# google/TensorNetwork

Hardware: NVIDIA H100
Metric: pairwise contractions/s (higher is better)
Workload: dtype bf16

## Files before the change

tensornetwork_b200/csrc/tensordot_thin.cu:

```cuda
#include "common.cuh"
#include <algorithm>
#include <vector>

namespace tnb {

struct ThinParams {
  const void* X; const void* S; void* C;
  int64_t L;
  int K, P;
  int64_t sXl, sXk;
  int64_t sCl;
  int64_t sSk;
  int64_t bX, bS, bC;
  int64_t batch;
  DevModes mP;
};

enum ThinKind { THIN_SIMT = 0, THIN_MMA = 1, THIN_MMA_TF32 = 2 };

template <typename T> struct Vec16 { static constexpr int N = 16 / (int)sizeof(T); };

__device__ __forceinline__ uint4 ldg16(const void* p) { return __ldg(reinterpret_cast<const uint4*>(p)); }

template <typename T> struct alignas(16) Pack16 { T v[Vec16<T>::N]; };

template <typename T, typename Acc, int KK, int PP>
__device__ __forceinline__ void simt_a_unit(const Acc (&w)[KK][PP], const Pack16<T> (&x)[KK], int K, int P, T* cp,
                                            const long long (&co)[PP]) {
  constexpr int VE = Vec16<T>::N;
  Acc acc[PP][VE];
#pragma unroll
  for (int i = 0; i < PP; ++i)
#pragma unroll
    for (int v = 0; v < VE; ++v) acc[i][v] = acc_zero((Acc*)nullptr);
#pragma unroll
  for (int k = 0; k < KK; ++k)
    if (k < K) {
#pragma unroll
      for (int v = 0; v < VE; ++v) {
        const Acc xv = to_acc(x[k].v[v]);
#pragma unroll
        for (int i = 0; i < PP; ++i) fma_acc(acc[i][v], w[k][i], xv);
      }
    }
#pragma unroll
  for (int i = 0; i < PP; ++i)
    if (i < P) {
      Pack16<T> o;
#pragma unroll
      for (int v = 0; v < VE; ++v) o.v[v] = FromAcc<T, Acc>::f(acc[i][v]);
      *reinterpret_cast<uint4*>(cp + co[i]) = *reinterpret_cast<uint4*>(&o);
    }
}

template <typename T, typename Acc, int KK, int PP>
__global__ void __launch_bounds__(256) thin_simt_a_kernel(const __grid_constant__ ThinParams p) {
  constexpr int VE = Vec16<T>::N;
  constexpr int U = (KK * PP <= 16) ? 2 : 1;
  __shared__ __align__(16) Acc sS[KK][PP];
  __shared__ long long cOff[PP];
  const int64_t bb = blockIdx.y;
  const T* Xb = (const T*)p.X + bb * p.bX;
  const T* Sb = (const T*)p.S + bb * p.bS;
  T* Cb = (T*)p.C + bb * p.bC;
  if (threadIdx.x < KK * PP) {
    const int k = threadIdx.x / PP, pp = threadIdx.x % PP;
    Acc v = acc_zero((Acc*)nullptr);
    if (pp < p.P) {
      int64_t os, oc;
      mode_offsets(p.mP, pp, os, oc);
      if (k < p.K) v = to_acc(Sb[os + k * p.sSk]);
      if (k == 0) cOff[pp] = oc;
    }
    sS[k][pp] = v;
  }
  __syncthreads();
  Acc w[KK][PP];
#pragma unroll
  for (int k = 0; k < KK; ++k)
#pragma unroll
    for (int i = 0; i < PP; ++i) w[k][i] = sS[k][i];
  long long co[PP];
#pragma unroll
  for (int i = 0; i < PP; ++i) co[i] = i < p.P ? cOff[i] : 0;
  const int64_t nunits = p.L / VE;
  const int64_t stride = (int64_t)gridDim.x * blockDim.x;
  for (int64_t u0 = blockIdx.x * (int64_t)blockDim.x + threadIdx.x; u0 < nunits; u0 += stride * U) {
    Pack16<T> x[U][KK];
#pragma unroll
    for (int j = 0; j < U; ++j)
      if (u0 + j * stride < nunits) {
        const T* xp = Xb + (u0 + j * stride) * VE;
#pragma unroll
        for (int k = 0; k < KK; ++k)
          if (k < p.K) *reinterpret_cast<uint4*>(&x[j][k]) = ldg16(xp + k * p.sXk);
      }
#pragma unroll
    for (int j = 0; j < U; ++j)
      if (u0 + j * stride < nunits) simt_a_unit<T, Acc, KK, PP>(w, x[j], p.K, p.P, Cb + (u0 + j * stride) * VE, co);
  }
}

template <typename T, int KK, int PP> struct SimtD {
  static constexpr int VE = Vec16<T>::N;
  static constexpr int UE = VE > KK ? VE : KK;
  static constexpr int R = UE / KK;
  static constexpr int NV = UE / VE;
  static constexpr int OE = R * PP;
  static constexpr int OB = OE * (int)sizeof(T);
};

template <typename T, typename Acc, int KK, int PP>
__device__ __forceinline__ void simt_d_unit(const Acc (&w)[KK][PP], const Pack16<T> (&x)[SimtD<T, KK, PP>::NV], T* cp) {
  using G = SimtD<T, KK, PP>;
  constexpr int VE = G::VE, R = G::R, OE = G::OE, OB = G::OB;
  struct alignas(OB >= 16 ? 16 : OB) Out { T v[OE]; };
  Out o;
#pragma unroll
  for (int r = 0; r < R; ++r) {
    Acc acc[PP];
#pragma unroll
    for (int j = 0; j < PP; ++j) acc[j] = acc_zero((Acc*)nullptr);
#pragma unroll
    for (int k = 0; k < KK; ++k) {
      const int e = r * KK + k;
      const Acc xv = to_acc(x[e / VE].v[e % VE]);
#pragma unroll
      for (int j = 0; j < PP; ++j) fma_acc(acc[j], xv, w[k][j]);
    }
#pragma unroll
    for (int j = 0; j < PP; ++j) o.v[r * PP + j] = FromAcc<T, Acc>::f(acc[j]);
  }
  if constexpr (OB >= 16) {
#pragma unroll
    for (int v = 0; v < OB / 16; ++v) reinterpret_cast<uint4*>(cp)[v] = reinterpret_cast<uint4*>(&o)[v];
  } else if constexpr (OB == 8) {
    *reinterpret_cast<uint2*>(cp) = *reinterpret_cast<uint2*>(&o);
  } else if constexpr (OB == 4) {
    *reinterpret_cast<uint32_t*>(cp) = *reinterpret_cast<uint32_t*>(&o);
  } else {
#pragma unroll
    for (int v = 0; v < OE; ++v) cp[v] = o.v[v];
  }
}

template <typename T, typename Acc, int KK, int PP>
__global__ void __launch_bounds__(256) thin_simt_d_kernel(const __grid_constant__ ThinParams p) {
  using G = SimtD<T, KK, PP>;
  constexpr int VE = G::VE, UE = G::UE, NV = G::NV, OE = G::OE;
  __shared__ Acc sS[KK][PP];
  const int64_t bb = blockIdx.y;
  const T* Xb = (const T*)p.X + bb * p.bX;
  const T* Sb = (const T*)p.S + bb * p.bS;
  T* Cb = (T*)p.C + bb * p.bC;
// ... 215 lines not shown
  const T* Sb = (const T*)p.S + bb * p.bS;
  T* Cb = (T*)p.C + bb * p.bC;
  for (int idx = threadIdx.x; idx < PP * KK; idx += blockDim.x) {
    const int pp = idx / KK, k = idx % KK;
    T v = FromAcc<T, float>::f(0.f);
    if (pp < p.P) {
      int64_t os, oc;
      mode_offsets(p.mP, pp, os, oc);
      v = Sb[os + k * p.sSk];
      if (k == 0) cOff[pp] = oc;
    }
    sS[pp * PITCH + k] = v;
  }
  __syncthreads();
  const int lane = threadIdx.x & 31, warp = threadIdx.x >> 5;
  const int g = lane >> 2, q = lane & 3;
  const int64_t nblk = p.L >> 6;
  const int64_t wstride = (int64_t)gridDim.x * (blockDim.x >> 5);

  if constexpr (MODE == 0) {
    uint32_t sa[PT][KT][4];
    mma_a_frags<T, KT, PT>(sS, sa, g, q);
    const int colbase = 32 * (g & 1) + 8 * (g >> 1);
    for (int64_t blk = (int64_t)blockIdx.x * (blockDim.x >> 5) + warp; blk < nblk; blk += wstride) {
      const int64_t l0 = blk << 6;
      mma_a_block<T, KT, PT, true>(sa, Xb + l0 + colbase, p.sXk, Cb + l0 + 8 * q, cOff, p.P, g, q);
    }
  } else {
    uint32_t sb[KT][2 * PT][2];
    mma_d_frags<T, KT, PT>(sS, sb, g, q);
    for (int64_t blk = (int64_t)blockIdx.x * (blockDim.x >> 5) + warp; blk < nblk; blk += wstride) {
      const int64_t l0 = blk << 6;
      mma_d_block<T, KT, PT, true>(sb, Xb + l0 * p.sXl, p.sXl, Cb + l0 * p.sCl, p.sCl, g, q);
    }
  }
}


__device__ __forceinline__ void mma_tf32(float (&d)[4], const uint32_t (&a)[4], uint32_t b0, uint32_t b1) {
  asm volatile("mma.sync.aligned.m16n8k8.row.col.f32.tf32.tf32.f32 {%0,%1,%2,%3}, {%4,%5,%6,%7}, {%8,%9}, {%0,%1,%2,%3};"
               : "+f"(d[0]), "+f"(d[1]), "+f"(d[2]), "+f"(d[3])
               : "r"(a[0]), "r"(a[1]), "r"(a[2]), "r"(a[3]), "r"(b0), "r"(b1));
}

template <int KT8, int PT, int MODE>
__global__ void __launch_bounds__(256) thin_mma32_kernel(const __grid_constant__ ThinParams p) {
  constexpr int KK = 8 * KT8, PP = 16 * PT, PITCH = KK + 4;
  __shared__ __align__(16) float sS[PP * PITCH];
  __shared__ long long cOff[PP];
  const int64_t bb = blockIdx.y;
  const float* Xb = (const float*)p.X + bb * p.bX;
  const float* Sb = (const float*)p.S + bb * p.bS;
  float* Cb = (float*)p.C + bb * p.bC;
  for (int idx = threadIdx.x; idx < PP * KK; idx += blockDim.x) {
    const int pp = idx / KK, k = idx % KK;
    float v = 0.f;
    if (pp < p.P) {
      int64_t os, oc;
      mode_offsets(p.mP, pp, os, oc);
      v = Sb[os + k * p.sSk];
      if (k == 0) cOff[pp] = oc;
    }
    sS[pp * PITCH + k] = v;
  }
  __syncthreads();
  const int lane = threadIdx.x & 31, warp = threadIdx.x >> 5;
  const int g = lane >> 2, q = lane & 3;
  const int64_t wstride = (int64_t)gridDim.x * (blockDim.x >> 5);

  if constexpr (MODE == 0) {
    const int64_t nblk = p.L >> 5;
    const int colbase = 16 * (g & 1) + 4 * (g >> 1);
    for (int64_t blk = (int64_t)blockIdx.x * (blockDim.x >> 5) + warp; blk < nblk; blk += wstride) {
      const int64_t l0 = blk << 5;
      const float* xp = Xb + l0 + colbase;
      uint4 x[KT8][2];
#pragma unroll
      for (int t = 0; t < KT8; ++t)
#pragma unroll
        for (int h = 0; h < 2; ++h) x[t][h] = ldg16(xp + (int64_t)(8 * t + q + 4 * h) * p.sXk);
#pragma unroll
      for (int mt = 0; mt < PT; ++mt) {
        if (16 * mt >= p.P) break;
        float acc[4][4];
#pragma unroll
        for (int j = 0; j < 4; ++j) { acc[j][0] = acc[j][1] = acc[j][2] = acc[j][3] = 0.f; }
#pragma unroll
        for (int t = 0; t < KT8; ++t) {
          const float* r0 = sS + (16 * mt + g) * PITCH + 8 * t + q;
          const uint32_t a[4] = {__float_as_uint(r0[0]), __float_as_uint(r0[8 * PITCH]), __float_as_uint(r0[4]),
                                 __float_as_uint(r0[8 * PITCH + 4])};
          mma_tf32(acc[0], a, x[t][0].x, x[t][1].x);
          mma_tf32(acc[1], a, x[t][0].y, x[t][1].y);
          mma_tf32(acc[2], a, x[t][0].z, x[t][1].z);
          mma_tf32(acc[3], a, x[t][0].w, x[t][1].w);
        }
#pragma unroll
        for (int h = 0; h < 2; ++h) {
          const int row = 16 * mt + g + 8 * h;
          if (row < p.P) {
            float* cp = Cb + cOff[row] + l0 + 4 * q;
            *reinterpret_cast<float4*>(cp) = make_float4(acc[0][2 * h], acc[1][2 * h], acc[2][2 * h], acc[3][2 * h]);
            *reinterpret_cast<float4*>(cp + 16) = make_float4(acc[0][2 * h + 1], acc[1][2 * h + 1], acc[2][2 * h + 1], acc[3][2 * h + 1]);
          }
        }
      }
    }
  } else {
    constexpr int NP8 = 2 * PT;
    constexpr int RG = KT8 == 8 ? 2 : 4;
    const int64_t nblk = p.L / (16 * RG);
    for (int64_t blk = (int64_t)blockIdx.x * (blockDim.x >> 5) + warp; blk < nblk; blk += wstride) {
      const int64_t l0 = blk * (16 * RG);
      uint32_t xa[RG][2][2 * KT8];
#pragma unroll
      for (int rg = 0; rg < RG; ++rg)
#pragma unroll
        for (int h = 0; h < 2; ++h) {
          const float* rp = Xb + (l0 + 16 * rg + 8 * h + g) * p.sXl + 2 * KT8 * q;
#pragma unroll
          for (int v4 = 0; v4 < KT8 / 2; ++v4) {
            const uint4 v = ldg16(rp + 4 * v4);
            xa[rg][h][4 * v4] = v.x; xa[rg][h][4 * v4 + 1] = v.y; xa[rg][h][4 * v4 + 2] = v.z; xa[rg][h][4 * v4 + 3] = v.w;
          }
        }
#pragma unroll
      for (int rg = 0; rg < RG; ++rg) {
        float acc[NP8][4];
#pragma unroll
        for (int pt = 0; pt < NP8; ++pt) { acc[pt][0] = acc[pt][1] = acc[pt][2] = acc[pt][3] = 0.f; }
#pragma unroll
        for (int t = 0; t < KT8; ++t) {
          const uint32_t a[4] = {xa[rg][0][2 * t], xa[rg][1][2 * t], xa[rg][0][2 * t + 1], xa[rg][1][2 * t + 1]};
#pragma unroll
          for (int pt = 0; pt < NP8; ++pt) {
            const int pcol = (pt >> 1) * 16 + 4 * (g >> 1) + 2 * (pt & 1) + (g & 1);
            const float2 b = *reinterpret_cast<const float2*>(sS + pcol * PITCH + 2 * KT8 * q + 2 * t);
            mma_tf32(acc[pt], a, __float_as_uint(b.x), __float_as_uint(b.y));
          }
        }
#pragma unroll
        for (int h = 0; h < 2; ++h) {
          float* cp = Cb + (l0 + 16 * rg + 8 * h + g) * p.sCl + 4 * q;
#pragma unroll
          for (int piece = 0; piece < NP8 / 2; ++piece)
            *reinterpret_cast<float4*>(cp + 16 * piece) =
                make_float4(acc[2 * piece][2 * h], acc[2 * piece][2 * h + 1], acc[2 * piece + 1][2 * h], acc[2 * piece + 1][2 * h + 1]);
        }
      }
    }
  }
}

constexpr int kRunMaxSteps = 8, kRunWarps = 8, kRunSlab = 4096;

struct ThinRunStep {
  const void* S; int64_t bS, sSk;
  int K, P, kind;
  int W;
  int64_t L;
  int soff;
};
struct ThinRunParams {
  const void* X; void* C;
  int64_t sX, bX;
  int64_t sC, bC;
  int64_t batch, nslab;
  int nsteps, smem_s;
  const long long* tab;
  ThinRunStep st[kRunMaxSteps];
};

__device__ __forceinline__ int run_pt(int P) { return (P + 15) / 16 <= 1 ? 1 : ((P + 15) / 16 <= 2 ? 2 : 4); }

__device__ __forceinline__ int64_t run_col(const ThinRunParams& p, int64_t slab, int n) {
  int64_t l = slab * 64;
  for (int j = p.nsteps - 2; j >= 0; --j) { l += (int64_t)(n / p.st[j].W) * p.st[j].L; n %= p.st[j].W; }
  return l + n;
}

template <typename T, int KT, int PT, int MODE>
__device__ __forceinline__ void run_mma(const ThinRunParams& p, int j, const unsigned char* smem, const long long* cOff,
                                        const T* x, int64_t sX, T* c, int64_t sC, bool last, int64_t slab, int g, int q) {
  const ThinRunStep& st = p.st[j];
  const T* sS = reinterpret_cast<const T*>(smem + st.soff);
  if constexpr (MODE == 0) {
    uint32_t sa[PT][KT][4];
    mma_a_frags<T, KT, PT>(sS, sa, g, q);
    const int colbase = 32 * (g & 1) + 8 * (g >> 1);
    for (int n0 = 0; n0 < st.W; n0 += 64)
      mma_a_block<T, KT, PT, false>(sa, x + n0 + colbase, sX, c + (last ? run_col(p, slab, n0) : n0) + 8 * q, cOff,
                                    st.P, g, q);
  } else {
    uint32_t sb[KT][2 * PT][2];
    mma_d_frags<T, KT, PT>(sS, sb, g, q);
    for (int n0 = 0; n0 < st.W; n0 += 64) mma_d_block<T, KT, PT, false>(sb, x + n0 * sX, sX, c + n0 * sC, sC, g, q);
  }
}

template <typename T, int KK, int PP, int MODE>
__device__ __forceinline__ void run_simt(const ThinRunParams& p, int j, const unsigned char* smem, const long long* cOff,
                                         const T* x, int64_t sX, T* c, bool last, int64_t slab, int lane) {
  using Acc = float;
  constexpr int VE = Vec16<T>::N;
  const ThinRunStep& st = p.st[j];
  const Acc* sS = reinterpret_cast<const Acc*>(smem + st.soff);
  Acc w[KK][PP];
#pragma unroll
  for (int k = 0; k < KK; ++k)
#pragma unroll
    for (int i = 0; i < PP; ++i) w[k][i] = sS[k * PP + i];
  if constexpr (MODE == 0) {
    long long co[PP];
#pragma unroll
    for (int i = 0; i < PP; ++i) co[i] = cOff[i];
    for (int u = lane; u < st.W / VE; u += 32) {
      Pack16<T> xv[KK];
#pragma unroll
      for (int k = 0; k < KK; ++k) *reinterpret_cast<uint4*>(&xv[k]) = ld16<false>(x + k * sX + u * VE);
      simt_a_unit<T, Acc, KK, PP>(w, xv, KK, PP, c + (last ? run_col(p, slab, u * VE) : u * VE), co);
    }
  } else {
    using G = SimtD<T, KK, PP>;
    for (int u = lane; u < st.W * KK / G::UE; u += 32) {
      Pack16<T> xv[G::NV];
#pragma unroll
      for (int v = 0; v < G::NV; ++v) *reinterpret_cast<uint4*>(&xv[v]) = ld16<false>(x + u * G::UE + v * VE);
      simt_d_unit<T, Acc, KK, PP>(w, xv, c + u * G::OE);
    }
  }
}

template <typename T, int MODE>
__global__ void __launch_bounds__(256, 1) thin_run_kernel(const __grid_constant__ ThinRunParams p) {
  extern __shared__ __align__(16) unsigned char smem[];
  long long* cOff = reinterpret_cast<long long*>(smem + p.smem_s);
  T* bufs = reinterpret_cast<T*>(cOff + kRunMaxSteps * 64);
  for (int i = threadIdx.x; i < p.nsteps * 64; i += blockDim.x) cOff[i] = p.tab[(i / 64) * 128 + 64 + i % 64];
  const int lane = threadIdx.x & 31, warp = threadIdx.x >> 5;
  const int g = lane >> 2, q = lane & 3;
  T* const wbuf = bufs + warp * 2 * kRunSlab;
  const int64_t total = p.batch * p.nslab;
  const int64_t beg = total * blockIdx.x / gridDim.x, end = total * (blockIdx.x + 1) / gridDim.x;
  for (int64_t s0 = beg; s0 < end;) {
    const int64_t b = s0 / p.nslab;
    const int64_t s1 = (b + 1) * p.nslab < end ? (b + 1) * p.nslab : end;
    __syncthreads();
    for (int j = 0; j < p.nsteps; ++j) {
      const ThinRunStep& st = p.st[j];
      const T* Sb = (const T*)st.S + b * st.bS;
      const long long* sOff = p.tab + j * 128;
      if (st.kind == THIN_MMA) {
        T* sS = reinterpret_cast<T*>(smem + st.soff);
        const int PP = 16 * run_pt(st.P), pitch = st.K + 8;
        for (int idx = threadIdx.x; idx < PP * st.K; idx += blockDim.x) {
          const int pp = idx / st.K, k = idx % st.K;
          sS[pp * pitch + k] = pp < st.P ? Sb[sOff[pp] + k * st.sSk] : FromAcc<T, float>::f(0.f);
        }
      } else {
        float* sS = reinterpret_cast<float*>(smem + st.soff);
        for (int idx = threadIdx.x; idx < st.K * st.P; idx += blockDim.x) {
          const int k = idx / st.P, pp = idx % st.P;
          sS[idx] = to_acc(Sb[sOff[pp] + k * st.sSk]);
        }
      }
    }
    __syncthreads();
    for (int64_t it = s0 + warp; it < s1; it += kRunWarps) {
      const int64_t slab = it - b * p.nslab;
      for (int j = 0; j < p.nsteps; ++j) {
        const ThinRunStep& st = p.st[j];
        const bool first = j == 0, last = j == p.nsteps - 1;
        const T* x = first ? (const T*)p.X + b * p.bX + slab * 64 * (MODE == 0 ? 1 : p.sX) : wbuf + ((j - 1) & 1) * kRunSlab;
        const int64_t sX = first ? p.sX : (MODE == 0 ? st.W : st.K);
        T* c = last ? (T*)p.C + b * p.bC + (MODE == 0 ? 0 : slab * st.W * p.sC) : wbuf + (j & 1) * kRunSlab;
        const int64_t sC = last ? p.sC : st.P;
        const long long* co = cOff + j * 64;
        if (st.kind == THIN_MMA) {
          const int kt = st.K / 16, pt = run_pt(st.P);
#define TNB_RUN_M(KT, PT) \
  if (kt == KT && pt == PT) run_mma<T, KT, PT, MODE>(p, j, smem, co, x, sX, c, sC, last, slab, g, q); else
          TNB_RUN_M(1, 1) TNB_RUN_M(1, 2) TNB_RUN_M(1, 4) TNB_RUN_M(2, 1) TNB_RUN_M(2, 2) TNB_RUN_M(2, 4)
          TNB_RUN_M(4, 1) TNB_RUN_M(4, 2) TNB_RUN_M(4, 4) {}
#undef TNB_RUN_M
        } else {
#define TNB_RUN_S(KK, PP) \
  if (st.K == KK && st.P == PP) run_simt<T, KK, PP, MODE>(p, j, smem, co, x, sX, c, last, slab, lane); else
          TNB_RUN_S(2, 2) TNB_RUN_S(2, 4) TNB_RUN_S(2, 8) TNB_RUN_S(4, 2) TNB_RUN_S(4, 4) TNB_RUN_S(4, 8)
          TNB_RUN_S(8, 2) TNB_RUN_S(8, 4) TNB_RUN_S(8, 8) {}
#undef TNB_RUN_S
        }
        __syncwarp();
      }
    }
    s0 = s1;
  }
}

static inline unsigned thin_grid_x(int64_t work_items, int64_t batch, int ctas_per_sm) {
  int64_t want = ((int64_t)num_sms() * ctas_per_sm + batch - 1) / batch;
  int64_t cap = (work_items + 255) / 256;
  if (want > cap) want = cap;
  if (want < 1) want = 1;
  return (unsigned)want;
}

template <int DT>
static int launch_simt(int mode, const ThinParams& p, cudaStream_t st) {
  using T = typename DType<DT>::T;
  using Acc = typename DType<DT>::Acc;
  constexpr int VE = 16 / (int)sizeof(T);
  if (mode == 0) {
    const int kk = p.K <= 2 ? 2 : (p.K <= 4 ? 4 : 8), pp = p.P <= 2 ? 2 : (p.P <= 4 ? 4 : 8);
    dim3 grid(thin_grid_x(p.L / VE, p.batch, 8), (unsigned)p.batch);
#define TNB_THIN_A(KK, PP) if (kk == KK && pp == PP) thin_simt_a_kernel<T, Acc, KK, PP><<<grid, 256, 0, st>>>(p);
    TNB_THIN_A(2, 2) TNB_THIN_A(2, 4) TNB_THIN_A(2, 8)
    TNB_THIN_A(4, 2) TNB_THIN_A(4, 4) TNB_THIN_A(4, 8)
    TNB_THIN_A(8, 2) TNB_THIN_A(8, 4) TNB_THIN_A(8, 8)
#undef TNB_THIN_A
    TNB_LAUNCH_CHECK();
    count_launch();
    set_kernel_name("thin_simt_a");
    return 0;
  }
#define TNB_THIN_D(KK, PP)                                                                         \
  if (p.K == KK && p.P == PP) {                                                                    \
    constexpr int UE = VE > KK ? VE : KK;                                                          \
    dim3 grid(thin_grid_x(p.L * KK / UE / 4, p.batch, 8), (unsigned)p.batch);                      \
    thin_simt_d_kernel<T, Acc, KK, PP><<<grid, 256, 0, st>>>(p);                                   \
    TNB_LAUNCH_CHECK();                                                                            \
    count_launch();                                                                                \
    set_kernel_name("thin_simt_d");                                                                \
    return 0;                                                                                      \
  }
  TNB_THIN_D(2, 2) TNB_THIN_D(2, 4) TNB_THIN_D(2, 8)
  TNB_THIN_D(4, 2) TNB_THIN_D(4, 4) TNB_THIN_D(4, 8)
  TNB_THIN_D(8, 2) TNB_THIN_D(8, 4) TNB_THIN_D(8, 8)
#undef TNB_THIN_D
  return TNB200_ERR_UNSUPPORTED;
}

template <int DT, int KT, int PT>
static int launch_mma_kp(int mode, const ThinParams& p, cudaStream_t st) {
  using T = typename DType<DT>::T;
  const int ctas = (KT * PT >= 8) ? 1 : (KT * PT >= 4 ? 2 : 4);
  int64_t want = ((int64_t)num_sms() * ctas + p.batch - 1) / p.batch;
  const int64_t cap = ((p.L >> 6) + 7) / 8;
  if (want > cap) want = cap;
  if (want < 1) want = 1;
  dim3 grid((unsigned)want, (unsigned)p.batch);
  if (mode == 0) thin_mma_kernel<T, KT, PT, 0><<<grid, 256, 0, st>>>(p);
  else thin_mma_kernel<T, KT, PT, 1><<<grid, 256, 0, st>>>(p);
  TNB_LAUNCH_CHECK();
  count_launch();
  set_kernel_name(mode == 0 ? "thin_mma_a" : "thin_mma_d");
  return 0;
}
template <int DT>
static int launch_mma(int mode, const ThinParams& p, cudaStream_t st) {
  const int kt = p.K / 16, pt = (p.P + 15) / 16 <= 1 ? 1 : ((p.P + 15) / 16 <= 2 ? 2 : 4);
#define TNB_THIN_M(KT, PT) if (kt == KT && pt == PT) return launch_mma_kp<DT, KT, PT>(mode, p, st);
  TNB_THIN_M(1, 1) TNB_THIN_M(1, 2) TNB_THIN_M(1, 4)
  TNB_THIN_M(2, 1) TNB_THIN_M(2, 2) TNB_THIN_M(2, 4)
  TNB_THIN_M(4, 1) TNB_THIN_M(4, 2) TNB_THIN_M(4, 4)
#undef TNB_THIN_M
  return TNB200_ERR_UNSUPPORTED;
}

template <int KT8, int PT>
static int launch_mma32_kp(int mode, const ThinParams& p, cudaStream_t st) {
  const int ctas = (KT8 * PT >= 16) ? 2 : 4;
  const int64_t nblk = mode == 0 ? (p.L >> 5) : p.L / (16 * (KT8 == 8 ? 2 : 4));
  int64_t want = ((int64_t)num_sms() * ctas + p.batch - 1) / p.batch;
  const int64_t cap = (nblk + 7) / 8;
  if (want > cap) want = cap;
  if (want < 1) want = 1;
  dim3 grid((unsigned)want, (unsigned)p.batch);
  if (mode == 0) thin_mma32_kernel<KT8, PT, 0><<<grid, 256, 0, st>>>(p);
  else thin_mma32_kernel<KT8, PT, 1><<<grid, 256, 0, st>>>(p);
  TNB_LAUNCH_CHECK();
  count_launch();
  set_kernel_name(mode == 0 ? "thin_mma_tf32_a" : "thin_mma_tf32_d");
  return 0;
}
static int launch_mma32(int mode, const ThinParams& p, cudaStream_t st) {
  const int kt = p.K / 8, pt = (p.P + 15) / 16 <= 1 ? 1 : ((p.P + 15) / 16 <= 2 ? 2 : 4);
#define TNB_THIN_M32(KT8, PT) if (kt == KT8 && pt == PT) return launch_mma32_kp<KT8, PT>(mode, p, st);
  TNB_THIN_M32(2, 1) TNB_THIN_M32(2, 2) TNB_THIN_M32(2, 4)
  TNB_THIN_M32(4, 1) TNB_THIN_M32(4, 2) TNB_THIN_M32(4, 4)
  TNB_THIN_M32(8, 1) TNB_THIN_M32(8, 2) TNB_THIN_M32(8, 4)
#undef TNB_THIN_M32
  return TNB200_ERR_UNSUPPORTED;
}

static inline bool al16(const void* p) { return ((uintptr_t)p & 15) == 0; }

static int plan_thin(int dt, const void* A, const void* B, void* C, const ModeList& mB, const ModeList& mM,
                     const ModeList& mN, const ModeList& mK, bool allow_tf32, ThinParams& p, int& mode, int& kind) {
  if (dt != TNB200_F64 && dt != TNB200_F32 && dt != TNB200_F16 && dt != TNB200_BF16) return TNB200_ERR_UNSUPPORTED;
  if (mB.n > 1 || mK.n != 1) return TNB200_ERR_UNSUPPORTED;
  const int64_t M = mM.total(), N = mN.total(), K = mK.total(), batch = mB.total();
  if (K > 64 || batch > 65535) return TNB200_ERR_UNSUPPORTED;
  const int64_t ve = 16 / dtype_size(dt);
  const bool half_t = dt == TNB200_F16 || dt == TNB200_BF16;
  memset(&p, 0, sizeof(p));
  p.K = (int)K; p.batch = batch;
  mode = -1;
  if (M <= 64 && mN.n == 1 && mN.s0[0] == 1 && mN.s1[0] == 1 && N >= 2048) {
    mode = 0;
    p.X = B; p.S = A; p.C = C; p.L = N; p.P = (int)M;
    p.sXl = 1; p.sXk = mK.s1[0]; p.sSk = mK.s0[0]; p.sCl = 1;
    p.bX = mB.n ? mB.s1[0] : 0; p.bS = mB.n ? mB.s0[0] : 0; p.bC = mB.n ? mB.s2[0] : 0;
    ModeList sp;
    for (int i = 0; i < mM.n; ++i) sp.push(mM.ext[i], mM.s0[i], mM.s1[i]);
    if (!to_dev(sp, p.mP)) return TNB200_ERR_UNSUPPORTED;
    bool ok = al16(B) && al16(C) && p.sXk % ve == 0 && p.bX % ve == 0 && p.bC % ve == 0;
    for (int i = 0; i < mM.n && ok; ++i) ok = mM.s1[i] % ve == 0;
    if (!ok) return TNB200_ERR_UNSUPPORTED;
  } else if (N <= 64 && mM.n == 1 && mK.s0[0] == 1 && M >= 2048) {
    int64_t run = 1;
    for (int i = mN.n - 1; i >= 0; --i) { if (mN.s1[i] != run) return TNB200_ERR_UNSUPPORTED; run *= mN.ext[i]; }
    mode = 1;
    p.X = A; p.S = B; p.C = C; p.L = M; p.P = (int)N;
    p.sXl = mM.s0[0]; p.sXk = 1; p.sSk = mK.s1[0]; p.sCl = mM.s1[0];
    p.bX = mB.n ? mB.s0[0] : 0; p.bS = mB.n ? mB.s1[0] : 0; p.bC = mB.n ? mB.s2[0] : 0;
    ModeList sp;
    for (int i = 0; i < mN.n; ++i) sp.push(mN.ext[i], mN.s0[i], mN.s1[i]);
    if (!to_dev(sp, p.mP)) return TNB200_ERR_UNSUPPORTED;
    if (!(al16(A) && al16(C) && p.bX % ve == 0 && p.bC % ve == 0)) return TNB200_ERR_UNSUPPORTED;
  } else {
    return TNB200_ERR_UNSUPPORTED;
  }
  if (p.L * batch < 65536) return TNB200_ERR_UNSUPPORTED;
  if (K <= 8 && p.P <= 8) {
    if (mode == 0) {
      if (p.L % ve) return TNB200_ERR_UNSUPPORTED;
    } else {
      const int64_t ue = ve > K ? ve : K;
      if (p.sXl != K || p.sCl != p.P || (p.L * K) % ue) return TNB200_ERR_UNSUPPORTED;
      if (!((K == 2 || K == 4 || K == 8) && (p.P == 2 || p.P == 4 || p.P == 8))) return TNB200_ERR_UNSUPPORTED;
    }
    kind = THIN_SIMT;
    return 0;
  }
  if (half_t && (K == 16 || K == 32 || K == 64) && p.P > 8 && p.L % 64 == 0) {
    if (mode == 1) {
      if (!(p.P == 16 || p.P == 32 || p.P == 64)) return TNB200_ERR_UNSUPPORTED;
      if (p.sXl % 8 || p.sCl % 8) return TNB200_ERR_UNSUPPORTED;
    }
    kind = THIN_MMA;
    return 0;
  }
  if (dt == TNB200_F32 && allow_tf32 && (K == 16 || K == 32 || K == 64) && p.P > 8) {
    if (mode == 0) {
      if (p.L % 32) return TNB200_ERR_UNSUPPORTED;
    } else {
      if (!(p.P == 16 || p.P == 32 || p.P == 64)) return TNB200_ERR_UNSUPPORTED;
      if (p.sXl % 4 || p.sCl % 4 || p.L % 64) return TNB200_ERR_UNSUPPORTED;
    }
    kind = THIN_MMA_TF32;
    return 0;
  }
  return TNB200_ERR_UNSUPPORTED;
}

int tensordot_thin(int dt, const void* A, const void* B, void* C, const ModeList& mB, const ModeList& mM,
                   const ModeList& mN, const ModeList& mK, bool allow_tf32, cudaStream_t st) {
  ThinParams p;
  int mode, kind;
  const int rc = plan_thin(dt, A, B, C, mB, mM, mN, mK, allow_tf32, p, mode, kind);
  if (rc) return rc;
  if (kind == THIN_MMA_TF32) return launch_mma32(mode, p, st);
  if (kind == THIN_MMA) return dt == TNB200_F16 ? launch_mma<TNB200_F16>(mode, p, st) : launch_mma<TNB200_BF16>(mode, p, st);
  switch (dt) {
    case TNB200_F64: return launch_simt<TNB200_F64>(mode, p, st);
    case TNB200_F32: return launch_simt<TNB200_F32>(mode, p, st);
    case TNB200_F16: return launch_simt<TNB200_F16>(mode, p, st);
    default: return launch_simt<TNB200_BF16>(mode, p, st);
  }
}

struct ThinRun {
  int dt, mode;
  ThinParams first, last;
  ThinRunParams rp;
  size_t smem;
  int grid;
};

static void host_mode_offsets(const DevModes& m, int64_t lin, int64_t& o0, int64_t& o1) {
  o0 = 0; o1 = 0;
  for (int i = m.n - 1; i > 0; --i) {
    const int64_t q = lin / m.ext[i], r = lin - q * m.ext[i];
    o0 += r * m.s0[i]; o1 += r * m.s1[i];
    lin = q;
  }
  if (m.n > 0) { o0 += lin * m.s0[0]; o1 += lin * m.s1[0]; }
}

template <typename T, int MODE> static void* thin_run_fn() { return (void*)thin_run_kernel<T, MODE>; }
static void* thin_run_kernel_ptr(int dt, int mode) {
  if (dt == TNB200_F16) return mode == 0 ? thin_run_fn<__half, 0>() : thin_run_fn<__half, 1>();
  return mode == 0 ? thin_run_fn<__nv_bfloat16, 0>() : thin_run_fn<__nv_bfloat16, 1>();
}

int thin_run_create(int dt, int nsteps, const ModeList* mB, const ModeList* mM, const ModeList* mN, const ModeList* mK,
                    const void* const* A, const void* const* B, void* const* C, const int* dep_a, const int* dep_b,
                    int* bad, void** handle) {
  *bad = -1;
  if (nsteps < 2 || nsteps > kRunMaxSteps) return TNB200_ERR_UNSUPPORTED;
  if (dt != TNB200_F16 && dt != TNB200_BF16) { *bad = 0; return TNB200_ERR_UNSUPPORTED; }
  std::vector<ThinParams> ps((size_t)nsteps);
  std::vector<long long> tab((size_t)nsteps * 128, 0);
  ThinRun* r = new ThinRun();
  memset(&r->rp, 0, sizeof(r->rp));
  r->dt = dt;
  int W = 64, soff = 0;
  auto fail = [&](int j) { *bad = j; delete r; return TNB200_ERR_UNSUPPORTED; };
  for (int j = 0; j < nsteps; ++j) {
    ThinParams& p = ps[j];
    int mode, kind;
    if (plan_thin(dt, A[j], B[j], C[j], mB[j], mM[j], mN[j], mK[j], false, p, mode, kind)) return fail(j);
    if (j == 0) r->mode = mode;
    if (mode != r->mode || (kind != THIN_SIMT && kind != THIN_MMA)) return fail(j);
    const int dep_x = mode == 0 ? dep_b[j] : dep_a[j], dep_s = mode == 0 ? dep_a[j] : dep_b[j];
    if (dep_s >= 0 || dep_x != j - 1) return fail(j);
    if (kind == THIN_SIMT && !((p.K == 2 || p.K == 4 || p.K == 8) && (p.P == 2 || p.P == 4 || p.P == 8))) return fail(j);
    if (j == 0 && p.L % 64) return fail(0);
    if (j > 0) {
      const ThinParams& pv = ps[j - 1];
      if (p.batch != pv.batch || p.L % pv.L) return fail(j);
      const int64_t R = p.L / pv.L;
      if ((int64_t)pv.P != p.K * R) return fail(j);
      if (r->mode == 0) {
        if (p.sXk < p.L) return fail(j);
        std::vector<char> seen((size_t)pv.P, 0);
        for (int pp = 0; pp < pv.P; ++pp) {
          int64_t os, oc;
          host_mode_offsets(pv.mP, pp, os, oc);
          const int64_t k = oc / p.sXk, rem = oc % p.sXk;
          if (rem % pv.L || rem / pv.L >= R || seen[k * R + rem / pv.L]) return fail(j);
          seen[k * R + rem / pv.L] = 1;
          tab[(size_t)(j - 1) * 128 + 64 + pp] = k * (W * R) + (rem / pv.L) * W;
        }
      } else if (p.sXl != p.K || pv.sCl != pv.P) {
        return fail(j);
      }
      W *= (int)R;
    }
    if ((int64_t)p.K * W > kRunSlab || (int64_t)p.P * W > kRunSlab) return fail(j);
    for (int pp = 0; pp < p.P; ++pp) {
      int64_t os, oc;
      host_mode_offsets(p.mP, pp, os, oc);
      tab[(size_t)j * 128 + pp] = os;
      if (j == nsteps - 1) tab[(size_t)j * 128 + 64 + pp] = oc;
    }
    ThinRunStep& st = r->rp.st[j];
    st.S = p.S; st.bS = p.bS; st.sSk = p.sSk; st.K = p.K; st.P = p.P; st.kind = kind; st.W = W; st.L = p.L;
    st.soff = soff;
    const int pt = (p.P + 15) / 16 <= 1 ? 1 : ((p.P + 15) / 16 <= 2 ? 2 : 4);
    soff += kind == THIN_MMA ? 16 * pt * (p.K + 8) * 2 : p.K * p.P * 4;
    soff = (soff + 15) / 16 * 16;
  }
  const ThinParams &p0 = ps[0], &pl = ps[nsteps - 1];
  ThinRunParams& rp = r->rp;
  rp.X = p0.X; rp.C = pl.C;
  rp.sX = r->mode == 0 ? p0.sXk : p0.sXl; rp.bX = p0.bX;
  rp.sC = pl.sCl; rp.bC = pl.bC;
  rp.batch = p0.batch; rp.nslab = p0.L / 64;
  rp.nsteps = nsteps; rp.smem_s = soff;
  r->smem = (size_t)soff + kRunMaxSteps * 64 * sizeof(long long) + (size_t)kRunWarps * 2 * kRunSlab * 2;
  void* fn = thin_run_kernel_ptr(dt, r->mode);
  int blocks = 0;
  constexpr int kRunSmemMax = kRunMaxSteps * 64 * (64 + 8) * 2 + kRunMaxSteps * 64 * (int)sizeof(long long) +
                              kRunWarps * 2 * kRunSlab * 2;
  if (cudaFuncSetAttribute(fn, cudaFuncAttributeMaxDynamicSharedMemorySize, kRunSmemMax) != cudaSuccess ||
      cudaOccupancyMaxActiveBlocksPerMultiprocessor(&blocks, fn, 256, r->smem) != cudaSuccess || blocks < 1) {
    cudaGetLastError();
    delete r;
    return TNB200_ERR_UNSUPPORTED;
  }
  const int64_t items = (rp.batch * rp.nslab + kRunWarps - 1) / kRunWarps;
  r->grid = (int)std::min<int64_t>((int64_t)blocks * num_sms(), items);
  long long* dtab = nullptr;
  if (cudaMalloc(&dtab, tab.size() * sizeof(long long)) != cudaSuccess ||
      cudaMemcpy(dtab, tab.data(), tab.size() * sizeof(long long), cudaMemcpyHostToDevice) != cudaSuccess) {
    cudaGetLastError();
    if (dtab) cudaFree(dtab);
    delete r;
    return TNB200_ERR_CUDA;
  }
  rp.tab = dtab;
  *handle = r;
  return 0;
}

int thin_run_launch(void* handle, cudaStream_t st) {
  const ThinRun* r = (const ThinRun*)handle;
  if (r->dt == TNB200_F16) {
    if (r->mode == 0) thin_run_kernel<__half, 0><<<r->grid, 256, r->smem, st>>>(r->rp);
    else thin_run_kernel<__half, 1><<<r->grid, 256, r->smem, st>>>(r->rp);
  } else {
    if (r->mode == 0) thin_run_kernel<__nv_bfloat16, 0><<<r->grid, 256, r->smem, st>>>(r->rp);
    else thin_run_kernel<__nv_bfloat16, 1><<<r->grid, 256, r->smem, st>>>(r->rp);
  }
  TNB_LAUNCH_CHECK();
  count_launch();
  set_kernel_name("thin_run");
  return 0;
}

int thin_run_destroy(void* handle) {
  ThinRun* r = (ThinRun*)handle;
  if (!r) return 0;
  cudaFree((void*)r->rp.tab);
  delete r;
  return 0;
}

}
```

Before: 1.158 million.

## Pipeline thin-run chain with cp.async prefetch, double-buffered S staging, and ramp specialization

Restructures the fused multi-step thin contraction kernel. Each warp's first-step input slab is now prefetched into shared memory with cp.async while the remaining chain steps of the previous slab run. The small S operands are staged for two batches at once when shared memory allows, which cuts block-wide barriers. A compile-time specialized 'ramp' variant is added for a K=64,32,16,8,4 halving chain, so dispatch and column-index math are resolved at compile time. This costs an extra warp buffer and more shared memory per block and more template instantiations, and it adds optional timing instrumentation behind a macro.

After: 1.173 million, median of 6. 1.01x the previous value.

```diff
diff --git a/tensornetwork_b200/csrc/tensordot_thin.cu b/tensornetwork_b200/csrc/tensordot_thin.cu
--- a/tensornetwork_b200/csrc/tensordot_thin.cu
+++ b/tensornetwork_b200/csrc/tensordot_thin.cu
@@ -1,5 +1,6 @@
 #include "common.cuh"
 #include <algorithm>
+#include <utility>
 #include <vector>
 
 namespace tnb {
@@ -521,7 +522,7 @@
   }
 }
 
-constexpr int kRunMaxSteps = 8, kRunWarps = 8, kRunSlab = 4096;
+constexpr int kRunMaxSteps = 8, kRunWarps = 8, kRunSlab = 4096, kRunBufs = 3;
 
 struct ThinRunStep {
   const void* S; int64_t bS, sSk;
@@ -536,19 +537,29 @@
   int64_t sC, bC;
   int64_t batch, nslab;
   int nsteps, smem_s;
+  int nsb;
   const long long* tab;
   ThinRunStep st[kRunMaxSteps];
 };
 
 __device__ __forceinline__ int run_pt(int P) { return (P + 15) / 16 <= 1 ? 1 : ((P + 15) / 16 <= 2 ? 2 : 4); }
 
+template <int RAMP>
 __device__ __forceinline__ int64_t run_col(const ThinRunParams& p, int64_t slab, int n) {
   int64_t l = slab * 64;
-  for (int j = p.nsteps - 2; j >= 0; --j) { l += (int64_t)(n / p.st[j].W) * p.st[j].L; n %= p.st[j].W; }
-  return l + n;
-}
-
-template <typename T, int KT, int PT, int MODE>
+  if constexpr (RAMP) {
+    constexpr int NS = __builtin_ctz(RAMP / 4) + 1;
+    for (int j = p.nsteps - 2; j >= NS - 1; --j) { l += (int64_t)(n / p.st[j].W) * p.st[j].L; n %= p.st[j].W; }
+#pragma unroll
+    for (int j = 0; j < NS - 1; ++j) l += (int64_t)((n >> (6 + j)) & 1) * p.st[j].L;
+    return l + (n & 63);
+  } else {
+    for (int j = p.nsteps - 2; j >= 0; --j) { l += (int64_t)(n / p.st[j].W) * p.st[j].L; n %= p.st[j].W; }
+    return l + n;
+  }
+}
+
+template <typename T, int KT, int PT, int MODE, int RAMP>
 __device__ __forceinline__ void run_mma(const ThinRunParams& p, int j, const unsigned char* smem, const long long* cOff,
                                         const T* x, int64_t sX, T* c, int64_t sC, bool last, int64_t slab, int g, int q) {
   const ThinRunStep& st = p.st[j];
@@ -558,7 +569,7 @@
     mma_a_frags<T, KT, PT>(sS, sa, g, q);
     const int colbase = 32 * (g & 1) + 8 * (g >> 1);
     for (int n0 = 0; n0 < st.W; n0 += 64)
-      mma_a_block<T, KT, PT, false>(sa, x + n0 + colbase, sX, c + (last ? run_col(p, slab, n0) : n0) + 8 * q, cOff,
+      mma_a_block<T, KT, PT, false>(sa, x + n0 + colbase, sX, c + (last ? run_col<RAMP>(p, slab, n0) : n0) + 8 * q, cOff,
                                     st.P, g, q);
   } else {
     uint32_t sb[KT][2 * PT][2];
@@ -567,7 +578,7 @@
   }
 }
 
-template <typename T, int KK, int PP, int MODE>
+template <typename T, int KK, int PP, int MODE, int RAMP>
 __device__ __forceinline__ void run_simt(const ThinRunParams& p, int j, const unsigned char* smem, const long long* cOff,
                                          const T* x, int64_t sX, T* c, bool last, int64_t slab, int lane) {
   using Acc = float;
@@ -587,7 +598,7 @@
       Pack16<T> xv[KK];
 #pragma unroll
       for (int k = 0; k < KK; ++k) *reinterpret_cast<uint4*>(&xv[k]) = ld16<false>(x + k * sX + u * VE);
-      simt_a_unit<T, Acc, KK, PP>(w, xv, KK, PP, c + (last ? run_col(p, slab, u * VE) : u * VE), co);
+      simt_a_unit<T, Acc, KK, PP>(w, xv, KK, PP, c + (last ? run_col<RAMP>(p, slab, u * VE) : u * VE), co);
     }
   } else {
     using G = SimtD<T, KK, PP>;
@@ -600,70 +611,185 @@
   }
 }
 
-template <typename T, int MODE>
+#ifdef TNB200_THIN_PHASES
+constexpr int kThinPhases = 6, kThinPhaseWarps = 4096;
+__device__ unsigned long long g_thin_phase[kThinPhaseWarps * kThinPhases];
+__device__ __forceinline__ unsigned long long thin_clock() {
+  unsigned long long t;
+  asm volatile("mov.u64 %0, %%globaltimer;" : "=l"(t)::"memory");
+  return t;
+}
+#define TNB_TPH(...) __VA_ARGS__
+#else
+#define TNB_TPH(...)
+#endif
+
+__device__ __forceinline__ void run_cp16(void* dst, const void* src) {
+  const uint32_t d = (uint32_t)__cvta_generic_to_shared(dst);
+  asm volatile("cp.async.cg.shared.global [%0], [%1], 16;" ::"r"(d), "l"(src) : "memory");
+}
+
+__device__ __forceinline__ int64_t run_first_item(int64_t s0, int64_t end, int64_t nslab, int warp) {
+  while (s0 < end) {
+    const int64_t s1 = (s0 / nslab + 1) * nslab < end ? (s0 / nslab + 1) * nslab : end;
+    if (s0 + warp < s1) return s0 + warp;
+    s0 = s1;
+  }
+  return end;
+}
+
+template <typename T, int MODE, int K0>
+__device__ __forceinline__ void run_prefetch(const ThinRunParams& p, int64_t it, T* slot, int lane) {
+  const int K = K0 ? K0 : p.st[0].K;
+  const int64_t b = it / p.nslab, slab = it - b * p.nslab;
+  const T* xb = (const T*)p.X + b * p.bX;
+  constexpr int VE = Vec16<T>::N;
+  const int nv = K * 64 / VE;
+  if constexpr (MODE == 0) {
+    for (int v = lane; v < nv; v += 32) {
+      const int k = v / (64 / VE), e = (v % (64 / VE)) * VE;
+      run_cp16(slot + k * 64 + e, xb + k * p.sX + slab * 64 + e);
+    }
+  } else if (!K0 && p.sX == K) {
+    const T* src = xb + slab * 64 * K;
+    for (int v = lane; v < nv; v += 32) run_cp16(slot + v * VE, src + v * VE);
+  } else {
+    for (int v = lane; v < nv; v += 32) {
+      const int r = v / (K / VE), e = (v % (K / VE)) * VE;
+      run_cp16(slot + r * K + e, xb + (slab * 64 + r) * p.sX + e);
+    }
+  }
+  asm volatile("cp.async.commit_group;" ::: "memory");
+}
+
+template <typename T, int MODE, int RAMP, int KC>
+__device__ __forceinline__ void run_step(const ThinRunParams& p, int j, const unsigned char* smem, const long long* cOff,
+                                         T* wbuf, int64_t b, int64_t slab, int lane) {
+  const int g = lane >> 2, q = lane & 3;
+  const ThinRunStep& st = p.st[j];
+  const bool last = j == p.nsteps - 1;
+  const T* x = wbuf + (j == 0 ? 0 : 1 + ((j - 1) & 1)) * kRunSlab;
+  const int64_t sX = MODE == 0 ? st.W : st.K;
+  T* c = last ? (T*)p.C + b * p.bC + (MODE == 0 ? 0 : slab * st.W * p.sC) : wbuf + (1 + (j & 1)) * kRunSlab;
+  const int64_t sC = last ? p.sC : st.P;
+  const long long* co = cOff + j * 64;
+  if constexpr (KC >= 16) {
+    run_mma<T, KC / 16, KC / 16, MODE, RAMP>(p, j, smem, co, x, sX, c, sC, last, slab, g, q);
+  } else if constexpr (KC > 0) {
+    run_simt<T, KC, KC, MODE, RAMP>(p, j, smem, co, x, sX, c, last, slab, lane);
+  } else if (KC == 0 && st.kind == THIN_MMA) {
+    if constexpr (KC == 0) {
+      const int kt = st.K / 16, pt = run_pt(st.P);
+#define TNB_RUN_M(KT, PT) \
+  if (kt == KT && pt == PT) run_mma<T, KT, PT, MODE, 0>(p, j, smem, co, x, sX, c, sC, last, slab, g, q); else
+      TNB_RUN_M(1, 1) TNB_RUN_M(1, 2) TNB_RUN_M(1, 4) TNB_RUN_M(2, 1) TNB_RUN_M(2, 2) TNB_RUN_M(2, 4)
+      TNB_RUN_M(4, 1) TNB_RUN_M(4, 2) TNB_RUN_M(4, 4) {}
+#undef TNB_RUN_M
+    }
+  } else {
+#define TNB_RUN_S(KK, PP) \
+  if (st.K == KK && st.P == PP) run_simt<T, KK, PP, MODE, RAMP>(p, j, smem, co, x, sX, c, last, slab, lane); else
+    TNB_RUN_S(2, 2) TNB_RUN_S(2, 4) TNB_RUN_S(2, 8) TNB_RUN_S(4, 2) TNB_RUN_S(4, 4) TNB_RUN_S(4, 8)
+    TNB_RUN_S(8, 2) TNB_RUN_S(8, 4) TNB_RUN_S(8, 8) {}
+#undef TNB_RUN_S
+  }
+  __syncwarp();
+}
+
+template <typename T, int MODE, int RAMP, int... J>
+__device__ __forceinline__ void run_ramp_rest(const ThinRunParams& p, const unsigned char* smem, const long long* cOff,
+                                              T* wbuf, int64_t b, int64_t slab, int lane, std::integer_sequence<int, J...>) {
+  (run_step<T, MODE, RAMP, (RAMP >> (J + 1))>(p, J + 1, smem, cOff, wbuf, b, slab, lane), ...);
+}
+
+template <typename T, int MODE, int RAMP>
 __global__ void __launch_bounds__(256, 1) thin_run_kernel(const __grid_constant__ ThinRunParams p) {
   extern __shared__ __align__(16) unsigned char smem[];
-  long long* cOff = reinterpret_cast<long long*>(smem + p.smem_s);
-  T* bufs = reinterpret_cast<T*>(cOff + kRunMaxSteps * 64);
-  for (int i = threadIdx.x; i < p.nsteps * 64; i += blockDim.x) cOff[i] = p.tab[(i / 64) * 128 + 64 + i % 64];
+  long long* cOff = reinterpret_cast<long long*>(smem + p.nsb * p.smem_s);
+  long long* sOffs = cOff + kRunMaxSteps * 64;
+  T* bufs = reinterpret_cast<T*>(sOffs + kRunMaxSteps * 64);
+  for (int i = threadIdx.x; i < p.nsteps * 64; i += blockDim.x) {
+    cOff[i] = p.tab[(i / 64) * 128 + 64 + i % 64];
+    sOffs[i] = p.tab[(i / 64) * 128 + i % 64];
+  }
   const int lane = threadIdx.x & 31, warp = threadIdx.x >> 5;
-  const int g = lane >> 2, q = lane & 3;
-  T* const wbuf = bufs + warp * 2 * kRunSlab;
+  T* const wbuf = bufs + warp * kRunBufs * kRunSlab;
   const int64_t total = p.batch * p.nslab;
   const int64_t beg = total * blockIdx.x / gridDim.x, end = total * (blockIdx.x + 1) / gridDim.x;
+  constexpr int K0 = RAMP;
+  {
+    const int64_t it = run_first_item(beg, end, p.nslab, warp);
+    if (it < end) run_prefetch<T, MODE, K0>(p, it, wbuf, lane);
+  }
+  TNB_TPH(unsigned long long ph[kThinPhases] = {0, 0, 0, 0, 0, 0}; unsigned long long t0 = thin_clock(), t1;)
+  int64_t staged = -1;
   for (int64_t s0 = beg; s0 < end;) {
     const int64_t b = s0 / p.nslab;
     const int64_t s1 = (b + 1) * p.nslab < end ? (b + 1) * p.nslab : end;
-    __syncthreads();
-    for (int j = 0; j < p.nsteps; ++j) {
-      const ThinRunStep& st = p.st[j];
-      const T* Sb = (const T*)st.S + b * st.bS;
-      const long long* sOff = p.tab + j * 128;
-      if (st.kind == THIN_MMA) {
-        T* sS = reinterpret_cast<T*>(smem + st.soff);
-        const int PP = 16 * run_pt(st.P), pitch = st.K + 8;
-        for (int idx = threadIdx.x; idx < PP * st.K; idx += blockDim.x) {
-          const int pp = idx / st.K, k = idx % st.K;
-          sS[pp * pitch + k] = pp < st.P ? Sb[sOff[pp] + k * st.sSk] : FromAcc<T, float>::f(0.f);
+    if (b > staged) {
+      __syncthreads();
+      const int64_t blast = (end - 1) / p.nslab;
+      for (int64_t bs = b; bs < b + p.nsb && bs <= blast; ++bs) {
+        unsigned char* sb = smem + ((bs - beg / p.nslab) % p.nsb) * p.smem_s;
+        for (int j = 0; j < p.nsteps; ++j) {
+          const ThinRunStep& st = p.st[j];
+          const T* Sb = (const T*)st.S + bs * st.bS;
+          const long long* sOff = sOffs + j * 64;
+          if (st.kind == THIN_MMA) {
+            T* sS = reinterpret_cast<T*>(sb + st.soff);
+            const int PP = 16 * run_pt(st.P), pitch = st.K + 8;
+#pragma unroll 8
+            for (int idx = threadIdx.x; idx < PP * st.K; idx += blockDim.x) {
+              const int pp = idx / st.K, k = idx % st.K;
+              sS[pp * pitch + k] = pp < st.P ? __ldg(Sb + sOff[pp] + k * st.sSk) : FromAcc<T, float>::f(0.f);
+            }
+          } else {
+            float* sS = reinterpret_cast<float*>(sb + st.soff);
+#pragma unroll 4
+            for (int idx = threadIdx.x; idx < st.K * st.P; idx += blockDim.x) {
+              const int k = idx / st.P, pp = idx % st.P;
+              sS[idx] = to_acc(__ldg(Sb + sOff[pp] + k * st.sSk));
+            }
+          }
+        }
+        staged = bs;
+      }
+      __syncthreads();
+    }
+    const unsigned char* sbuf = smem + ((b - beg / p.nslab) % p.nsb) * p.smem_s;
+    TNB_TPH(t1 = thin_clock(); ph[4] += t1 - t0; t0 = t1;)
+    for (int64_t it = s0 + warp; it < s1; it += kRunWarps) {
+      const int64_t slab = it - b * p.nslab;
+      asm volatile("cp.async.wait_group 0;" ::: "memory");
+      __syncwarp();
+      TNB_TPH(t1 = thin_clock(); ph[0] += t1 - t0; t0 = t1;)
+      run_step<T, MODE, RAMP, K0>(p, 0, sbuf, cOff, wbuf, b, slab, lane);
+      TNB_TPH(t1 = thin_clock(); ph[1] += t1 - t0; t0 = t1;)
+      const int64_t nx = it + kRunWarps < s1 ? it + kRunWarps : run_first_item(s1, end, p.nslab, warp);
+      if (nx < end) run_prefetch<T, MODE, K0>(p, nx, wbuf, lane);
+      if constexpr (RAMP) {
+        constexpr int NS = __builtin_ctz(RAMP / 4) + 1;
+        run_ramp_rest<T, MODE, RAMP>(p, sbuf, cOff, wbuf, b, slab, lane, std::make_integer_sequence<int, NS - 2>{});
+        if (p.nsteps == NS) {
+          TNB_TPH(t1 = thin_clock(); ph[2] += t1 - t0; t0 = t1;)
+          run_step<T, MODE, RAMP, 4>(p, NS - 1, sbuf, cOff, wbuf, b, slab, lane);
+        } else {
+          run_step<T, MODE, RAMP, 4>(p, NS - 1, sbuf, cOff, wbuf, b, slab, lane);
+          for (int j = NS; j < p.nsteps - 1; ++j) run_step<T, MODE, RAMP, -1>(p, j, sbuf, cOff, wbuf, b, slab, lane);
+          TNB_TPH(t1 = thin_clock(); ph[2] += t1 - t0; t0 = t1;)
+          run_step<T, MODE, RAMP, -1>(p, p.nsteps - 1, sbuf, cOff, wbuf, b, slab, lane);
         }
       } else {
-        float* sS = reinterpret_cast<float*>(smem + st.soff);
-        for (int idx = threadIdx.x; idx < st.K * st.P; idx += blockDim.x) {
-          const int k = idx / st.P, pp = idx % st.P;
-          sS[idx] = to_acc(Sb[sOff[pp] + k * st.sSk]);
-        }
+        for (int j = 1; j < p.nsteps - 1; ++j) run_step<T, MODE, 0, 0>(p, j, sbuf, cOff, wbuf, b, slab, lane);
+        TNB_TPH(t1 = thin_clock(); ph[2] += t1 - t0; t0 = t1;)
+        run_step<T, MODE, 0, 0>(p, p.nsteps - 1, sbuf, cOff, wbuf, b, slab, lane);
       }
-    }
-    __syncthreads();
-    for (int64_t it = s0 + warp; it < s1; it += kRunWarps) {
-      const int64_t slab = it - b * p.nslab;
-      for (int j = 0; j < p.nsteps; ++j) {
-        const ThinRunStep& st = p.st[j];
-        const bool first = j == 0, last = j == p.nsteps - 1;
-        const T* x = first ? (const T*)p.X + b * p.bX + slab * 64 * (MODE == 0 ? 1 : p.sX) : wbuf + ((j - 1) & 1) * kRunSlab;
-        const int64_t sX = first ? p.sX : (MODE == 0 ? st.W : st.K);
-        T* c = last ? (T*)p.C + b * p.bC + (MODE == 0 ? 0 : slab * st.W * p.sC) : wbuf + (j & 1) * kRunSlab;
-        const int64_t sC = last ? p.sC : st.P;
-        const long long* co = cOff + j * 64;
-        if (st.kind == THIN_MMA) {
-          const int kt = st.K / 16, pt = run_pt(st.P);
-#define TNB_RUN_M(KT, PT) \
-  if (kt == KT && pt == PT) run_mma<T, KT, PT, MODE>(p, j, smem, co, x, sX, c, sC, last, slab, g, q); else
-          TNB_RUN_M(1, 1) TNB_RUN_M(1, 2) TNB_RUN_M(1, 4) TNB_RUN_M(2, 1) TNB_RUN_M(2, 2) TNB_RUN_M(2, 4)
-          TNB_RUN_M(4, 1) TNB_RUN_M(4, 2) TNB_RUN_M(4, 4) {}
-#undef TNB_RUN_M
-        } else {
-#define TNB_RUN_S(KK, PP) \
-  if (st.K == KK && st.P == PP) run_simt<T, KK, PP, MODE>(p, j, smem, co, x, sX, c, last, slab, lane); else
-          TNB_RUN_S(2, 2) TNB_RUN_S(2, 4) TNB_RUN_S(2, 8) TNB_RUN_S(4, 2) TNB_RUN_S(4, 4) TNB_RUN_S(4, 8)
-          TNB_RUN_S(8, 2) TNB_RUN_S(8, 4) TNB_RUN_S(8, 8) {}
-#undef TNB_RUN_S
-        }
-        __syncwarp();
-      }
+      TNB_TPH(t1 = thin_clock(); ph[3] += t1 - t0; t0 = t1; ph[5] += 1;)
     }
     s0 = s1;
   }
+  TNB_TPH(const int slot = blockIdx.x * kRunWarps + warp;
+          if (lane == 0 && slot < kThinPhaseWarps) for (int i = 0; i < kThinPhases; ++i) g_thin_phase[slot * kThinPhases + i] += ph[i];)
 }
 
 static inline unsigned thin_grid_x(int64_t work_items, int64_t batch, int ctas_per_sm) {
@@ -851,6 +977,7 @@
 
 struct ThinRun {
   int dt, mode;
+  int ramp;
   ThinParams first, last;
   ThinRunParams rp;
   size_t smem;
@@ -867,10 +994,13 @@
   if (m.n > 0) { o0 += lin * m.s0[0]; o1 += lin * m.s1[0]; }
 }
 
-template <typename T, int MODE> static void* thin_run_fn() { return (void*)thin_run_kernel<T, MODE>; }
-static void* thin_run_kernel_ptr(int dt, int mode) {
-  if (dt == TNB200_F16) return mode == 0 ? thin_run_fn<__half, 0>() : thin_run_fn<__half, 1>();
-  return mode == 0 ? thin_run_fn<__nv_bfloat16, 0>() : thin_run_fn<__nv_bfloat16, 1>();
+template <typename T, int MODE, int RAMP> static void* thin_run_fn() { return (void*)thin_run_kernel<T, MODE, RAMP>; }
+template <typename T, int RAMP> static void* thin_run_fn(int mode) {
+  return mode == 0 ? thin_run_fn<T, 0, RAMP>() : thin_run_fn<T, 1, RAMP>();
+}
+static void* thin_run_kernel_ptr(int dt, int mode, int ramp) {
+  if (dt == TNB200_F16) return ramp ? thin_run_fn<__half, 64>(mode) : thin_run_fn<__half, 0>(mode);
+  return ramp ? thin_run_fn<__nv_bfloat16, 64>(mode) : thin_run_fn<__nv_bfloat16, 0>(mode);
 }
 
 int thin_run_create(int dt, int nsteps, const ModeList* mB, const ModeList* mM, const ModeList* mN, const ModeList* mK,
@@ -937,13 +1067,23 @@
   rp.sX = r->mode == 0 ? p0.sXk : p0.sXl; rp.bX = p0.bX;
   rp.sC = pl.sCl; rp.bC = pl.bC;
   rp.batch = p0.batch; rp.nslab = p0.L / 64;
-  rp.nsteps = nsteps; rp.smem_s = soff;
-  r->smem = (size_t)soff + kRunMaxSteps * 64 * sizeof(long long) + (size_t)kRunWarps * 2 * kRunSlab * 2;
-  void* fn = thin_run_kernel_ptr(dt, r->mode);
-  int blocks = 0;
-  constexpr int kRunSmemMax = kRunMaxSteps * 64 * (64 + 8) * 2 + kRunMaxSteps * 64 * (int)sizeof(long long) +
-                              kRunWarps * 2 * kRunSlab * 2;
-  if (cudaFuncSetAttribute(fn, cudaFuncAttributeMaxDynamicSharedMemorySize, kRunSmemMax) != cudaSuccess ||
+  rp.nsteps = nsteps; rp.smem_s = soff; rp.nsb = 1;
+  r->smem = (size_t)soff + 2 * kRunMaxSteps * 64 * sizeof(long long) + (size_t)kRunWarps * kRunBufs * kRunSlab * 2;
+  r->ramp = nsteps >= 5 ? 64 : 0;
+  for (int j = 0; j < 5 && r->ramp; ++j) {
+    const ThinRunStep& st = rp.st[j];
+    if (st.K != 64 >> j || st.P != st.K || st.W != 64 << j || st.kind != (j < 3 ? THIN_MMA : THIN_SIMT)) r->ramp = 0;
+  }
+  void* fn = thin_run_kernel_ptr(dt, r->mode, r->ramp);
+  int blocks = 0, smem_max = 0, dev = 0;
+  if (cudaGetDevice(&dev) == cudaSuccess &&
+      cudaDeviceGetAttribute(&smem_max, cudaDevAttrMaxSharedMemoryPerBlockOptin, dev) == cudaSuccess &&
+      r->smem + soff <= (size_t)smem_max) {
+    rp.nsb = 2;
+    r->smem += soff;
+  }
+  if (smem_max == 0 || r->smem > (size_t)smem_max ||
+      cudaFuncSetAttribute(fn, cudaFuncAttributeMaxDynamicSharedMemorySize, smem_max) != cudaSuccess ||
       cudaOccupancyMaxActiveBlocksPerMultiprocessor(&blocks, fn, 256, r->smem) != cudaSuccess || blocks < 1) {
     cudaGetLastError();
     delete r;
@@ -966,13 +1106,9 @@
 
 int thin_run_launch(void* handle, cudaStream_t st) {
   const ThinRun* r = (const ThinRun*)handle;
-  if (r->dt == TNB200_F16) {
-    if (r->mode == 0) thin_run_kernel<__half, 0><<<r->grid, 256, r->smem, st>>>(r->rp);
-    else thin_run_kernel<__half, 1><<<r->grid, 256, r->smem, st>>>(r->rp);
-  } else {
-    if (r->mode == 0) thin_run_kernel<__nv_bfloat16, 0><<<r->grid, 256, r->smem, st>>>(r->rp);
-    else thin_run_kernel<__nv_bfloat16, 1><<<r->grid, 256, r->smem, st>>>(r->rp);
-  }
+  const void* fn = thin_run_kernel_ptr(r->dt, r->mode, r->ramp);
+  void* args[] = {(void*)&r->rp};
+  cudaLaunchKernel(fn, dim3(r->grid), dim3(256), args, r->smem, st);
   TNB_LAUNCH_CHECK();
   count_launch();
   set_kernel_name("thin_run");
@@ -988,3 +1124,15 @@
 }
 
 }
+
+#ifdef TNB200_THIN_PHASES
+extern "C" TNB200_API int32_t tnb200_thin_phases(unsigned long long* out, int32_t reset) {
+  if (cudaMemcpyFromSymbol(out, tnb::g_thin_phase, sizeof(tnb::g_thin_phase)) != cudaSuccess) return TNB200_ERR_CUDA;
+  if (reset) {
+    void* p = nullptr;
+    if (cudaGetSymbolAddress(&p, tnb::g_thin_phase) != cudaSuccess || cudaMemset(p, 0, sizeof(tnb::g_thin_phase)) != cudaSuccess)
+      return TNB200_ERR_CUDA;
+  }
+  return 0;
+}
+#endif
```
